# zhengfei0908/SBA-GAN

Measured on AMD Instinct MI355X. Metric: images/sec (G+D step) at 256px, higher is better.
Workload: dtype bf16; 1 GPU; bird_style.yml 3-stage G+D step (64..256px), B=20 per GPU, G_NET variant=model, image_encoder=inception, text_encoder=RNN_ENCODER in the step; global_batch=20, parallelism=dp1, launch=replayer, losses_finite=True

## Files before the change

### sba-gan_amd/csrc/norm_act.hip

```cpp
#include "common.h"

namespace {

constexpr float LRELU_SLOPE = 0.2f;


template <int ACT>
__device__ __forceinline__ float bn_act_elem(float ya, float sca, float sha, float yg, float scg, float shg) {
    const float n = ya * sca + sha;
    if (ACT == SBA_ACT_GLU) return n * sigmoidf_(yg * scg + shg);
    if (ACT == SBA_ACT_LRELU) return n > 0.f ? n : LRELU_SLOPE * n;
    if (ACT == SBA_ACT_RELU) return fmaxf(n, 0.f);
    return n;
}

struct ChCoef { float scale, shift, mean, rstd; };
__device__ __forceinline__ void ch_coef_pair(const float* __restrict__ scale, const float* __restrict__ shift,
                                             const float* __restrict__ mean, const float* __restrict__ rstd, int ca, int cg,
                                             ChCoef& ka, ChCoef& kg) {
    ka.scale = scale[ca]; ka.shift = shift[ca]; kg.scale = scale[cg]; kg.shift = shift[cg];
    ka.mean = mean[ca]; ka.rstd = rstd[ca]; kg.mean = mean[cg]; kg.rstd = rstd[cg];
}
template <int ACT>
__device__ __forceinline__ void bn_bwd_elem(float ya, float yg, float dd, const ChCoef& ka, const ChCoef& kg,
                                            float (&dz)[2], float (&xh)[2]) {
    if (ACT == SBA_ACT_GLU) {
        const float n = ya * ka.scale + ka.shift;
        const float gp = yg * kg.scale + kg.shift;
        const float s = sigmoid_bwd_(gp);
        dz[0] = dd * s;
        dz[1] = dd * n * s * (1.f - s);
    } else {
        dz[0] = dd;
        if (ACT == SBA_ACT_LRELU) {
            const float n = ya * ka.scale + ka.shift;
            dz[0] = n > 0.f ? dd : LRELU_SLOPE * dd;
        }
    }
    xh[0] = (ya - ka.mean) * ka.rstd;
    if (ACT == SBA_ACT_GLU) xh[1] = (yg - kg.mean) * kg.rstd;
}

struct Moments { float mean, var, rstd; };
__device__ __forceinline__ Moments moments_of(float sum, float sumsq, float count, float eps) {
    Moments m;
    m.mean = sum / count;
    m.var = fmaxf(sumsq / count - m.mean * m.mean, 0.f);
    m.rstd = rsqrtf(m.var + eps);
    return m;
}
struct BnCoef { float scale, shift, mean, rstd, var; };
__device__ __forceinline__ BnCoef bn_affine(float mean, float var, float rstd, float gamma, float beta) {
    BnCoef k;
    k.mean = mean; k.var = var; k.rstd = rstd;
    k.scale = gamma * rstd;
    k.shift = beta - mean * k.scale;
    return k;
}
__device__ __forceinline__ void store_aux(float* __restrict__ aux, int C, int c, const BnCoef& k) {
    aux[c] = k.scale; aux[C + c] = k.shift; aux[2 * C + c] = k.mean; aux[3 * C + c] = k.rstd;
}
__device__ __forceinline__ void running_update(float& rm, float& rv, float mean, float var, float count, float momentum) {
    const float unb = count > 1.f ? var * count / (count - 1.f) : var;
    rm = (1.f - momentum) * rm + momentum * mean;
    rv = (1.f - momentum) * rv + momentum * unb;
}
__device__ __forceinline__ BnCoef bn_coef(const float* __restrict__ stats, const float* __restrict__ gamma,
                                          const float* __restrict__ beta, int C, int c, float count, float eps) {
    float s0 = 0.f, s1 = 0.f;
#pragma unroll
    for (int sl = 0; sl < SBA_BN_STAT_SLOTS; ++sl) {
        s0 += stats[sl * 2 * C + c];
        s1 += stats[sl * 2 * C + C + c];
    }
    const Moments m = moments_of(s0, s1, count, eps);
    return bn_affine(m.mean, m.var, m.rstd, gamma[c], beta[c]);
}

struct ChannelSum {
    float* acc;
    int C;
    bool det;
    __device__ __forceinline__ void clear() const {
        if (det) return;
        for (int i = threadIdx.x; i < 2 * C; i += blockDim.x) acc[i] = 0.f;
        __syncthreads();
    }
    template <int V>
    __device__ __forceinline__ void add(int tr, int c, const float (&s0)[V], const float (&s1)[V]) const {
        float* row = acc + (det ? tr * 2 * C : 0);
#pragma unroll
        for (int k = 0; k < V; ++k) {
            if (det) {
                row[c + k] = s0[k];
                row[C + c + k] = s1[k];
            } else {
                atomicAdd(&row[c + k], s0[k]);
                atomicAdd(&row[C + c + k], s1[k]);
            }
        }
    }
    template <typename Dst>
    __device__ __forceinline__ void finish(int rpi, Dst dst) const {
        __syncthreads();
        for (int i = threadIdx.x; i < 2 * C; i += blockDim.x) {
            float v = det ? 0.f : acc[i];
            if (det)
                for (int r = 0; r < rpi; ++r) v += acc[r * 2 * C + i];
            dst(i, v);
        }
    }
};

template <int NV, int V>
__device__ __forceinline__ void wave_sums_to_lds(const float (&s0)[NV][V], const float (&s1)[NV][V],
                                                 float (&s_red)[4][2 * NV * V]) {
    const int lane = threadIdx.x & 63, wid = threadIdx.x >> 6;
#pragma unroll
    for (int h = 0; h < NV; ++h)
#pragma unroll
        for (int k = 0; k < V; ++k) {
            const float a0 = wave_sum(s0[h][k]), a1 = wave_sum(s1[h][k]);
            if (lane == 0) { s_red[wid][(h * V + k) * 2] = a0; s_red[wid][(h * V + k) * 2 + 1] = a1; }
        }
    __syncthreads();
}
template <int W>
__device__ __forceinline__ float four_wave_sum(const float (&s_red)[4][W], int i) {
    return s_red[0][i] + s_red[1][i] + s_red[2][i] + s_red[3][i];
}

template <typename T>
__global__ __launch_bounds__(256) void bn_stats_kernel(const T* __restrict__ y_all, float* __restrict__ stats_all, int64_t rows, int C,
                                                       float* __restrict__ det_part) {
    constexpr int V = Vec16<T>::N;
    const T* y = y_all + (int64_t)blockIdx.y * rows * C;
    float* stats = stats_all + ((int64_t)blockIdx.y * SBA_BN_STAT_SLOTS + (blockIdx.x & (SBA_BN_STAT_SLOTS - 1))) * 2 * C;
    const int cv = C / V;
    extern __shared__ float s_acc[];
    const ChannelSum cs{s_acc, C, det_part != nullptr};
    cs.clear();
    const int tpr = cv < (int)blockDim.x ? cv : (int)blockDim.x;
    const int rpi = blockDim.x / tpr;
    const int tc = threadIdx.x % tpr, tr = threadIdx.x / tpr;
    for (int cvi = tc; cvi < cv && tr < rpi; cvi += tpr) {
        const int c = cvi * V;
        float s0[V], s1[V];
#pragma unroll
        for (int k = 0; k < V; ++k) s0[k] = s1[k] = 0.f;
        for (int64_t row = (int64_t)blockIdx.x * rpi + tr; row < rows; row += (int64_t)gridDim.x * rpi) {
            Vec16<T> a = ld16(y + row * C + c);
#pragma unroll
            for (int k = 0; k < V; ++k) { const float v = a.get(k); s0[k] += v; s1[k] += v * v; }
        }
        cs.add(tr, c, s0, s1);
    }
    float* part = det_part ? det_part + ((int64_t)blockIdx.y * gridDim.x + blockIdx.x) * 2 * C : nullptr;
    cs.finish(rpi, [&](int i, float v) {
        if (det_part) part[i] = v;
        else atomicAdd(&stats[i], v);
    });
}

template <typename T, typename YT, int ACT>
__global__ __launch_bounds__(256) void bn_act_fwd_kernel(const YT* __restrict__ y_all, const float* __restrict__ stats_all,
                                  const float* __restrict__ gamma, const float* __restrict__ beta,
                                  float* __restrict__ rmean, float* __restrict__ rvar, int64_t* __restrict__ nbt,
                                  float* __restrict__ aux_all, const T* __restrict__ residual_all,
                                  T* __restrict__ out_all, int64_t rows, int C, int out_cstride, int out_coff,
                                  float eps, float momentum, int training) {
    constexpr int V = Vec16<T>::N;
    extern __shared__ float s_co[];
    const int g = blockIdx.y;
    const int Co = ACT == SBA_ACT_GLU ? C / 2 : C;
    const float count = (float)rows;
    float* aux = aux_all + (int64_t)g * 4 * C;
    for (int c = threadIdx.x; c < C; c += blockDim.x) {
        BnCoef k;
        if (training) {
            k = bn_coef(stats_all + (int64_t)g * SBA_BN_STAT_SLOTS * 2 * C, gamma, beta, C, c, count, eps);
        } else {
            k = bn_affine(rmean[c], rvar[c], rsqrtf(rvar[c] + eps), gamma[c], beta[c]);
        }
        s_co[c] = k.scale;
        s_co[C + c] = k.shift;
        if (blockIdx.x == 0) store_aux(aux, C, c, k);
        if (blockIdx.x == 0 && g == 0 && training && rmean) {
            float rm = rmean[c], rv = rvar[c];
            for (int gg = 0; gg < (int)gridDim.y; ++gg) {
                const BnCoef q = bn_coef(stats_all + (int64_t)gg * SBA_BN_STAT_SLOTS * 2 * C, gamma, beta, C, c, count, eps);
                running_update(rm, rv, q.mean, q.var, count, momentum);
            }
            rmean[c] = rm;
            rvar[c] = rv;
        }
    }
    if (blockIdx.x == 0 && g == 0 && threadIdx.x == 0 && training && nbt) *nbt += gridDim.y;
    __syncthreads();
    const float* scale = s_co;
    const float* shift = s_co + C;
    const YT* y = y_all + (int64_t)g * rows * C;
    const T* residual = ACT != SBA_ACT_GLU && residual_all ? residual_all + (int64_t)g * rows * Co : nullptr;
    T* out = out_all + (int64_t)g * rows * out_cstride;
    const int cv = Co / V;
    const int64_t total = rows * cv;
    for (int64_t i = blockIdx.x * (int64_t)blockDim.x + threadIdx.x; i < total;
         i += (int64_t)gridDim.x * blockDim.x) {
        const int64_t row = i / cv;
        const int c = (int)(i - row * cv) * V;
        Vec16<YT> a = ld16(y + row * C + c);
        Vec16<YT> gt = ACT == SBA_ACT_GLU ? ld16(y + row * C + Co + c) : a;
        Vec16<T> r, o;
        if (residual) r = ld16(residual + row * Co + c);
// ... 107 lines not shown
        }
        return;
    }
    for (int i = threadIdx.x; i < 2 * C; i += blockDim.x) atomicAdd(&red[i], s_acc[i]);
}

template <typename T, typename YT, int ACT>
__global__ __launch_bounds__(256) void bn_bwd_apply_kernel(const YT* __restrict__ y_all, const T* __restrict__ dout_all,
                                    const float* __restrict__ aux_all, const float* __restrict__ red_all,
                                    T* __restrict__ dy_all, float* __restrict__ dgamma, float* __restrict__ dbeta,
                                    int64_t rows, int C, int dcs, int dco) {
    constexpr int V = Vec16<T>::N;
    extern __shared__ float s_k[];
    const int g = blockIdx.y;
    const float* aux = aux_all + (int64_t)g * 4 * C;
    const float* red = red_all + (int64_t)g * SBA_BN_STAT_SLOTS * 2 * C;
    const float inv = 1.f / (float)rows;
    for (int c = threadIdx.x; c < C; c += blockDim.x) {
        s_k[c] = aux[c]; s_k[C + c] = aux[C + c]; s_k[2 * C + c] = aux[2 * C + c]; s_k[3 * C + c] = aux[3 * C + c];
        float r0 = 0.f, r1 = 0.f;
#pragma unroll
        for (int sl = 0; sl < SBA_BN_STAT_SLOTS; ++sl) {
            r0 += red[(int64_t)sl * 2 * C + c];
            r1 += red[(int64_t)sl * 2 * C + C + c];
        }
        s_k[4 * C + c] = r0 * inv;
        s_k[5 * C + c] = r1 * inv;
        if (blockIdx.x == 0 && dgamma) {
            atomicAdd(&dgamma[c], r1);
            atomicAdd(&dbeta[c], r0);
        }
    }
    __syncthreads();
    const float* scale = s_k;
    const float* shift = s_k + C;
    const float* mean = s_k + 2 * C;
    const float* rstd = s_k + 3 * C;
    const float* P = s_k + 4 * C;
    const float* Q = s_k + 5 * C;
    const YT* y = y_all + (int64_t)g * rows * C;
    const T* dout = dout_all + (int64_t)g * rows * dcs;
    T* dy = dy_all + (int64_t)g * rows * C;
    const int Co = ACT == SBA_ACT_GLU ? C / 2 : C;
    const int cv = Co / V;
    const int64_t total = rows * cv;
    for (int64_t i = blockIdx.x * (int64_t)blockDim.x + threadIdx.x; i < total;
         i += (int64_t)gridDim.x * blockDim.x) {
        const int64_t row = i / cv;
        const int c = (int)(i - row * cv) * V;
        Vec16<YT> a = ld16(y + row * C + c);
        Vec16<T> d = ld16(dout + row * dcs + dco + c);
        Vec16<T> o;
        if (ACT == SBA_ACT_GLU) {
            Vec16<YT> gt = ld16(y + row * C + Co + c);
            Vec16<T> og;
#pragma unroll
            for (int k = 0; k < V; ++k) {
                const int ca = c + k, cg = Co + c + k;
                float dz[2], xh[2];
                ChCoef ka, kg;
                ch_coef_pair(scale, shift, mean, rstd, ca, cg, ka, kg);
                bn_bwd_elem<ACT>(a.get(k), gt.get(k), d.get(k), ka, kg, dz, xh);
                o.set(k, scale[ca] * (dz[0] - P[ca] - xh[0] * Q[ca]));
                og.set(k, scale[cg] * (dz[1] - P[cg] - xh[1] * Q[cg]));
            }
            st16(dy + row * C + Co + c, og);
        } else {
#pragma unroll
            for (int k = 0; k < V; ++k) {
                const int ca = c + k;
                float dz = d.get(k);
                if (ACT == SBA_ACT_LRELU) {
                    const float n = a.get(k) * scale[ca] + shift[ca];
                    dz = n > 0.f ? dz : LRELU_SLOPE * dz;
                }
                const float xa = (a.get(k) - mean[ca]) * rstd[ca];
                o.set(k, scale[ca] * (dz - P[ca] - xa * Q[ca]));
            }
        }
        st16(dy + row * C + c, o);
    }
}

template <typename T, typename YT, int ACT>
__global__ __launch_bounds__(256) void bn_fwd_fused_kernel(const YT* __restrict__ y_all, const float* __restrict__ gamma,
                                                           const float* __restrict__ beta, float* __restrict__ rmean,
                                                           float* __restrict__ rvar, int64_t* __restrict__ nbt,
                                                           float* __restrict__ aux_all, T* __restrict__ out_all,
                                                           int64_t rows, int groups, int C, int out_cstride,
                                                           int out_coff, float eps, float momentum) {
    constexpr int V = Vec16<T>::N;
    constexpr int NV = ACT == SBA_ACT_GLU ? 2 : 1;
    __shared__ float s_red[4][2 * NV * V];
    __shared__ float s_co[2 * NV * V];
    const int tid = threadIdx.x;
    const int Co = ACT == SBA_ACT_GLU ? C / 2 : C;
    const int c = blockIdx.x * V;
    const float count = (float)rows;
    if (blockIdx.x == 0 && tid == 0 && nbt) *nbt += groups;
    for (int g = 0; g < groups; ++g) {
        const YT* y = y_all + (int64_t)g * rows * C;
        T* out = out_all + (int64_t)g * rows * out_cstride;
        float* aux = aux_all + (int64_t)g * 4 * C;
        float s0[NV][V], s1[NV][V];
#pragma unroll
        for (int h = 0; h < NV; ++h)
#pragma unroll
            for (int k = 0; k < V; ++k) { s0[h][k] = 0.f; s1[h][k] = 0.f; }
        for (int64_t row = tid; row < rows; row += 256) {
#pragma unroll
            for (int h = 0; h < NV; ++h) {
                Vec16<YT> a = ld16(y + row * C + c + h * Co);
#pragma unroll
                for (int k = 0; k < V; ++k) { const float v = a.get(k); s0[h][k] += v; s1[h][k] += v * v; }
            }
        }
        wave_sums_to_lds(s0, s1, s_red);
        if (tid < NV * V) {
            const int h = tid / V, k = tid - h * V, ch = c + h * Co + k;
            const Moments m = moments_of(four_wave_sum(s_red, tid * 2), four_wave_sum(s_red, tid * 2 + 1), count, eps);
            const BnCoef q = bn_affine(m.mean, m.var, m.rstd, gamma[ch], beta[ch]);
            s_co[tid * 2] = q.scale;
            s_co[tid * 2 + 1] = q.shift;
            store_aux(aux, C, ch, q);
            if (rmean) running_update(rmean[ch], rvar[ch], q.mean, q.var, count, momentum);
        }
        __syncthreads();
        for (int64_t row = tid; row < rows; row += 256) {
            Vec16<YT> a = ld16(y + row * C + c);
            Vec16<YT> gt = ACT == SBA_ACT_GLU ? ld16(y + row * C + Co + c) : a;
            Vec16<T> o;
#pragma unroll
            for (int k = 0; k < V; ++k) {
                const int kg = (NV - 1) * V + k;
                o.set(k, bn_act_elem<ACT>(a.get(k), s_co[k * 2], s_co[k * 2 + 1], gt.get(k), s_co[kg * 2], s_co[kg * 2 + 1]));
            }
            st16(out + row * out_cstride + out_coff + c, o);
        }
        __syncthreads();
    }
}

template <typename T, typename YT, int ACT>
__global__ __launch_bounds__(256) void bn_bwd_fused_kernel(const YT* __restrict__ y_all, const T* __restrict__ dout_all,
                                                           const float* __restrict__ aux_all, T* __restrict__ dy_all,
                                                           float* __restrict__ dgamma, float* __restrict__ dbeta,
                                                           int64_t rows, int C, int dcs, int dco) {
    constexpr int V = Vec16<T>::N;
    constexpr int NV = ACT == SBA_ACT_GLU ? 2 : 1;
    __shared__ float s_red[4][2 * NV * V];
    __shared__ float s_tot[2 * NV * V];
    const int g = blockIdx.y, tid = threadIdx.x;
    const int Co = ACT == SBA_ACT_GLU ? C / 2 : C;
    const int c = blockIdx.x * V;
    const YT* y = y_all + (int64_t)g * rows * C;
    const T* dout = dout_all + (int64_t)g * rows * dcs;
    T* dy = dy_all + (int64_t)g * rows * C;
    const float* aux = aux_all + (int64_t)g * 4 * C;
    ChCoef kc[NV][V];
#pragma unroll
    for (int k = 0; k < V; ++k)
        ch_coef_pair(aux, aux + C, aux + 2 * C, aux + 3 * C, c + k, c + (NV - 1) * Co + k, kc[0][k], kc[NV - 1][k]);
    float s0[NV][V], s1[NV][V];
#pragma unroll
    for (int h = 0; h < NV; ++h)
#pragma unroll
        for (int k = 0; k < V; ++k) { s0[h][k] = 0.f; s1[h][k] = 0.f; }
    auto dz_row = [&](int64_t row, float (&dz)[NV][V], float (&xh)[NV][V]) {
        Vec16<YT> a = ld16(y + row * C + c);
        Vec16<T> d = ld16(dout + row * dcs + dco + c);
        Vec16<YT> gt = ACT == SBA_ACT_GLU ? ld16(y + row * C + Co + c) : a;
#pragma unroll
        for (int k = 0; k < V; ++k) {
            float z[2], x[2];
            bn_bwd_elem<ACT>(a.get(k), gt.get(k), d.get(k), kc[0][k], kc[NV - 1][k], z, x);
#pragma unroll
            for (int h = 0; h < NV; ++h) { dz[h][k] = z[h]; xh[h][k] = x[h]; }
        }
    };
    for (int64_t row = tid; row < rows; row += 256) {
        float dz[NV][V], xh[NV][V];
        dz_row(row, dz, xh);
#pragma unroll
        for (int h = 0; h < NV; ++h)
#pragma unroll
            for (int k = 0; k < V; ++k) { s0[h][k] += dz[h][k]; s1[h][k] += dz[h][k] * xh[h][k]; }
    }
    wave_sums_to_lds(s0, s1, s_red);
    if (tid < 2 * NV * V) s_tot[tid] = four_wave_sum(s_red, tid);
    __syncthreads();
    if (tid < NV * V && dgamma) {
        const int h = tid / V, k = tid - h * V;
        atomicAdd(&dgamma[c + h * Co + k], s_tot[tid * 2 + 1]);
        atomicAdd(&dbeta[c + h * Co + k], s_tot[tid * 2]);
    }
    const float inv = 1.f / (float)rows;
    for (int64_t row = tid; row < rows; row += 256) {
        float dz[NV][V], xh[NV][V];
        dz_row(row, dz, xh);
#pragma unroll
        for (int h = 0; h < NV; ++h) {
            Vec16<T> o;
#pragma unroll
            for (int k = 0; k < V; ++k)
                o.set(k, kc[h][k].scale * (dz[h][k] - s_tot[(h * V + k) * 2] * inv - xh[h][k] * s_tot[(h * V + k) * 2 + 1] * inv));
            st16(dy + row * C + c + h * Co, o);
        }
    }
}

constexpr int BN1D_BM = 32;
template <bool CACHED, typename T, int N>
__device__ __forceinline__ float sample_at(const float (&cache)[N], const T* __restrict__ p, int stride, int col, int b) {
    if constexpr (CACHED) return cache[b];
    else return to_f<T>(p[(int64_t)b * stride + col]);
}
#define BN1D_EACH_SAMPLE(b, B, CACHED) \
    _Pragma("unroll CACHED ? BN1D_BM : 1") for (int b = 0; b < (CACHED ? BN1D_BM : B); ++b) if (b < B)

template <typename T, bool CACHED>
__device__ __forceinline__ void bn1d_glu_fwd_body(const float* __restrict__ y, const float* __restrict__ gamma,
                                                  const float* __restrict__ beta, float* __restrict__ rmean,
                                                  float* __restrict__ rvar, float* __restrict__ mean_o,
                                                  float* __restrict__ rstd_o, T* __restrict__ out, int B, int F, int f,
                                                  float eps, float momentum) {
    const int fh = F / 2, Cg = fh / 16;
    float yv[2][CACHED ? BN1D_BM : 1];
    if constexpr (CACHED) {
#pragma unroll
        for (int b = 0; b < BN1D_BM; ++b) {
            yv[0][b] = b < B ? y[(int64_t)b * F + f] : 0.f;
            yv[1][b] = b < B ? y[(int64_t)b * F + f + fh] : 0.f;
        }
    }
    float sc[2], sh[2];
#pragma unroll
    for (int h = 0; h < 2; ++h) {
        const int ff = f + h * fh;
        float s = 0.f, q = 0.f;
        BN1D_EACH_SAMPLE(b, B, CACHED) s += sample_at<CACHED>(yv[h], y, F, ff, b);
        const float mean = s / B;
        BN1D_EACH_SAMPLE(b, B, CACHED) { const float v = sample_at<CACHED>(yv[h], y, F, ff, b) - mean; q += v * v; }
        const float var = q / B, r = rsqrtf(var + eps);
        sc[h] = gamma[ff] * r; sh[h] = beta[ff] - mean * sc[h];
        mean_o[ff] = mean; rstd_o[ff] = r;
        if (rmean) running_update(rmean[ff], rvar[ff], mean, var, (float)B, momentum);
    }
    const int c = f / 16, s16 = f % 16;
    BN1D_EACH_SAMPLE(b, B, CACHED) {
        const float ya = sample_at<CACHED>(yv[0], y, F, f, b), yg = sample_at<CACHED>(yv[1], y, F, f + fh, b);
        const float n = fmaf(ya, sc[0], sh[0]), gp = fmaf(yg, sc[1], sh[1]);
        out[((int64_t)b * 16 + s16) * Cg + c] = from_f<T>(n * sigmoidf_(gp));
    }
}

template <typename T>
__global__ __launch_bounds__(256) void bn1d_glu_fwd_kernel(const float* __restrict__ y, const float* __restrict__ gamma,
                                    const float* __restrict__ beta, float* __restrict__ rmean,
                                    float* __restrict__ rvar, int64_t* __restrict__ nbt,
                                    float* __restrict__ mean_o, float* __restrict__ rstd_o,
                                    T* __restrict__ out, int B, int F, float eps, float momentum) {
    const int f = blockIdx.x * blockDim.x + threadIdx.x;
    if (f == 0 && nbt) *nbt += 1;
    if (f >= F / 2) return;
    if (B <= BN1D_BM) bn1d_glu_fwd_body<T, true>(y, gamma, beta, rmean, rvar, mean_o, rstd_o, out, B, F, f, eps, momentum);
    else bn1d_glu_fwd_body<T, false>(y, gamma, beta, rmean, rvar, mean_o, rstd_o, out, B, F, f, eps, momentum);
}

struct Bn1dCoef { float scale, beta, mean, rstd; };
__device__ __forceinline__ void bn1d_glu_dz(float ya, float yg, float dd, const Bn1dCoef& ka, const Bn1dCoef& kg,
                                            float& dza, float& dzg) {
    const float n = (ya - ka.mean) * ka.scale + ka.beta, gp = (yg - kg.mean) * kg.scale + kg.beta, s = sigmoidf_(gp);
    dza = dd * s;
    dzg = dd * n * s * (1.f - s);
}

template <typename T, bool CACHED>
__device__ __forceinline__ void bn1d_glu_bwd_body(const float* __restrict__ y, const T* __restrict__ dout,
                                                  const float* __restrict__ gamma, const float* __restrict__ beta,
                                                  const float* __restrict__ mean, const float* __restrict__ rstd,
                                                  float* __restrict__ dy, float* __restrict__ dgamma,
                                                  float* __restrict__ dbeta, int B, int F, int f) {
    const int fh = F / 2, Cg = fh / 16;
    const int fa = f, fg = f + fh, dcol = (f % 16) * Cg + f / 16;
    const Bn1dCoef ka{gamma[fa] * rstd[fa], beta[fa], mean[fa], rstd[fa]}, kg{gamma[fg] * rstd[fg], beta[fg], mean[fg], rstd[fg]};
    constexpr int NB = CACHED ? BN1D_BM : 1;
    float ya_[NB], yg_[NB], dd_[NB];
    if constexpr (CACHED) {
// ... 71 lines not shown
    const int n = blockIdx.x, tc = blockIdx.y, tid = threadIdx.x;
    const T* base = h + (int64_t)n * HW * C + tc * V;
    float s0[V], s1[V];
#pragma unroll
    for (int k = 0; k < V; ++k) s0[k] = s1[k] = 0.f;
    int p = tid;
    for (; p + 3 * 256 < HW; p += 4 * 256) {
        Vec16<T> a0 = ld16(base + (int64_t)p * C), a1 = ld16(base + (int64_t)(p + 256) * C);
        Vec16<T> a2 = ld16(base + (int64_t)(p + 512) * C), a3 = ld16(base + (int64_t)(p + 768) * C);
#pragma unroll
        for (int k = 0; k < V; ++k) {
            const float v0 = a0.get(k), v1 = a1.get(k), v2 = a2.get(k), v3 = a3.get(k);
            s0[k] += (v0 + v1) + (v2 + v3);
            s1[k] += (v0 * v0 + v1 * v1) + (v2 * v2 + v3 * v3);
        }
    }
    for (; p < HW; p += 256) {
        Vec16<T> a = ld16(base + (int64_t)p * C);
#pragma unroll
        for (int k = 0; k < V; ++k) { const float v = a.get(k); s0[k] += v; s1[k] += v * v; }
    }
    __shared__ float s_part[4][2 * V];
#pragma unroll
    for (int k = 0; k < V; ++k) {
        const float a = wave_sum(s0[k]), b = wave_sum(s1[k]);
        if ((tid & 63) == 0) { s_part[tid >> 6][k] = a; s_part[tid >> 6][V + k] = b; }
    }
    __syncthreads();
    if (tid < V) {
        const float sm = (s_part[0][tid] + s_part[1][tid]) + (s_part[2][tid] + s_part[3][tid]);
        const float sq = (s_part[0][V + tid] + s_part[1][V + tid]) + (s_part[2][V + tid] + s_part[3][V + tid]);
        const Moments m = moments_of(sm, sq, (float)HW, eps);
        mean[n * C + tc * V + tid] = m.mean;
        rstd[n * C + tc * V + tid] = m.rstd;
    }
}

__global__ __launch_bounds__(256) void instnorm_finalize_kernel(float* __restrict__ mean, float* __restrict__ rstd, int NC,
                                         float HW, float eps) {
    const int i = blockIdx.x * blockDim.x + threadIdx.x;
    if (i >= NC) return;
    const Moments m = moments_of(mean[i], rstd[i], HW, eps);
    mean[i] = m.mean;
    rstd[i] = m.rstd;
}

template <typename T>
__global__ __launch_bounds__(256) void adain_fwd_kernel(const T* __restrict__ h, const float* __restrict__ mean,
                                 const float* __restrict__ rstd, const float* __restrict__ style,
                                 T* __restrict__ out, int N, int HW, int C, int ocs, int oco) {
    constexpr int V = Vec16<T>::N;
    const int cv = C / V;
    const int64_t total = (int64_t)N * HW * cv;
    for (int64_t i = blockIdx.x * (int64_t)blockDim.x + threadIdx.x; i < total;
         i += (int64_t)gridDim.x * blockDim.x) {
        const int64_t row = i / cv;
        const int c = (int)(i - row * cv) * V;
        const int n = (int)(row / HW);
        Vec16<T> a = ld16(h + row * C + c), o;
#pragma unroll
        for (int k = 0; k < V; ++k) {
            const float xh = (a.get(k) - mean[n * C + c + k]) * rstd[n * C + c + k];
            o.set(k, (style[n * 2 * C + c + k] + 1.f) * xh + style[n * 2 * C + C + c + k]);
        }
        st16(out + row * ocs + oco + c, o);
    }
}

template <typename T>
__global__ __launch_bounds__(256) void adain_bwd_reduce_kernel(const T* __restrict__ h, const T* __restrict__ dout,
                                        const float* __restrict__ mean, const float* __restrict__ rstd,
                                        float* __restrict__ red, int HW, int C, int dcs, int dco, int det) {
    constexpr int V = Vec16<T>::N;
    const int cv = C / V, n = blockIdx.x;
    const int rpi = blockDim.x / cv;
    const int tc = threadIdx.x % cv, tr = threadIdx.x / cv;
    extern __shared__ float s_acc[];
    const ChannelSum cs{s_acc, C, det != 0};
    cs.clear();
    float s0[V], s1[V];
#pragma unroll
    for (int k = 0; k < V; ++k) s0[k] = s1[k] = 0.f;
    if (tr < rpi) {
        for (int p = blockIdx.y * rpi + tr; p < HW; p += gridDim.y * rpi) {
            const int64_t row = (int64_t)n * HW + p;
            Vec16<T> a = ld16(h + row * C + tc * V);
            Vec16<T> d = ld16(dout + row * dcs + dco + tc * V);
#pragma unroll
            for (int k = 0; k < V; ++k) {
                const int c = tc * V + k;
                const float xh = (a.get(k) - mean[n * C + c]) * rstd[n * C + c];
                s0[k] += d.get(k) * xh;
                s1[k] += d.get(k);
            }
        }
        cs.add(tr, tc * V, s0, s1);
    }
    cs.finish(rpi, [&](int i, float v) {
        float* dst = i < C ? &red[(n * C + i) * 2 + 0] : &red[(n * C + i - C) * 2 + 1];
        if (det) *dst += v;
        else atomicAdd(dst, v);
    });
}

template <typename T>
__global__ __launch_bounds__(256) void adain_bwd_apply_kernel(const T* __restrict__ h, const T* __restrict__ dout,
                                       const float* __restrict__ mean, const float* __restrict__ rstd,
                                       const float* __restrict__ style, const float* __restrict__ red,
                                       T* __restrict__ dh, float* __restrict__ dstyle, int N, int HW,
                                       int C, int dcs, int dco, int accumulate) {
    constexpr int V = Vec16<T>::N;
    const int cv = C / V;
    const float inv = 1.f / HW;
    if (blockIdx.x == 0 && dstyle) {
        for (int i = threadIdx.x; i < N * C; i += blockDim.x) {
            const int n = i / C, c = i - n * C;
            dstyle[n * 2 * C + c] = red[i * 2 + 0];
            dstyle[n * 2 * C + C + c] = red[i * 2 + 1];
        }
    }
    const int64_t total = (int64_t)N * HW * cv;
    for (int64_t i = blockIdx.x * (int64_t)blockDim.x + threadIdx.x; i < total;
         i += (int64_t)gridDim.x * blockDim.x) {
        const int64_t row = i / cv;
        const int c = (int)(i - row * cv) * V;
        const int n = (int)(row / HW);
        Vec16<T> a = ld16(h + row * C + c);
        Vec16<T> d = ld16(dout + row * dcs + dco + c);
        Vec16<T> o;
        if (accumulate) o = ld16(dh + row * C + c);
#pragma unroll
        for (int k = 0; k < V; ++k) {
            const int nc = n * C + c + k;
            const float xh = (a.get(k) - mean[nc]) * rstd[nc];
            const float g = (style[n * 2 * C + c + k] + 1.f) * rstd[nc];
            float v = g * (d.get(k) - red[nc * 2 + 1] * inv - xh * red[nc * 2 + 0] * inv);
            if (accumulate) v += o.get(k);
            o.set(k, v);
        }
        st16(dh + row * C + c, o);
    }
}

inline int grid_for(int64_t items, int cap = 4096) {
    int64_t b = (items + 255) / 256;
    if (b < 1) b = 1;
    return (int)(b > cap ? cap : b);
}
inline bool pow2(int v) { return v > 0 && (v & (v - 1)) == 0; }

inline int vec_width(int dtype) { return dtype != SBA_F32 ? 8 : 4; }
inline int64_t elem_size(int dtype) { return dtype != SBA_F32 ? 2 : 4; }
inline bool slice_ok(int stride, int offset, int width, int V) {
    return stride >= width + offset && stride % V == 0 && offset % V == 0;
}
inline int act_width(int C, int act) { return act == SBA_ACT_GLU ? C / 2 : C; }

constexpr int BN_RED_WORKGROUPS = 512;
constexpr int BN_RED_WORKGROUPS_PER_GROUP = 64;
struct ReduceGrid { int rpi, blocks; };
inline ReduceGrid reduce_grid(int64_t rows, int cv, int groups) {
    ReduceGrid r;
    r.rpi = cv < 256 ? 256 / cv : 1;
    r.blocks = cdiv(rows, (int64_t)r.rpi * 8);
    const int cap = BN_RED_WORKGROUPS / groups > BN_RED_WORKGROUPS_PER_GROUP ? BN_RED_WORKGROUPS / groups
                                                                              : BN_RED_WORKGROUPS_PER_GROUP;
    if (r.blocks > cap) r.blocks = cap;
    if (r.blocks < 1) r.blocks = 1;
    return r;
}
template <typename Launch>
int reduce_pass(int groups, ReduceGrid rg, int C, float* dst, hipStream_t st, Launch launch) {
    float* part = nullptr;
    size_t sh = 2 * (size_t)C * sizeof(float);
    if (sba_det_on()) {
        part = sba_det_alloc((int64_t)groups * rg.blocks * 2 * C);
        if (!part) return SBA_E_ARG;
        sh *= rg.rpi;
    }
    const int rc = launch(sh, part);
    if (rc != SBA_OK) return rc;
    if (part) sba_det_fold(part, groups, rg.blocks, 2 * C, dst, (int64_t)SBA_BN_STAT_SLOTS * 2 * C, 0, st);
    return SBA_CHECK_LAUNCH();
}
template <typename Launch>
int param_grad_pass(int groups, bool param_grads, Launch launch) {
    const int step = sba_det_on() && groups > 1 && param_grads ? 1 : groups;
    for (int g = 0; g < groups; g += step) {
        const int rc = launch(g, step);
        if (rc != SBA_OK) return rc;
    }
    return SBA_CHECK_LAUNCH();
}
inline int instnorm_splits(int HW, int rpi, bool det) {
    const int splits = cdiv(HW, rpi * 16);
    return det ? 1 : splits > 256 ? 256 : splits;
}

}

extern "C" int sba_bn_stats(int dtype, const void* y, float* stats, int64_t rows, int groups, int C,
                            void* stream) {
    const int V = vec_width(dtype);
    if (!y || !stats || rows <= 0 || groups <= 0 || groups > 65535 || C <= 0 || C % V || C > 4096)
        return SBA_E_ARG;
    const ReduceGrid rg = reduce_grid(rows, C / V, groups);
    return reduce_pass(groups, rg, C, stats, (hipStream_t)stream, [&](size_t sh, float* part) -> int {
        SBA_DISPATCH_Y(dtype, SBA_LAUNCH((bn_stats_kernel<YT>), dim3(rg.blocks, groups), dim3(256), sh, (hipStream_t)stream,
                                         (const YT*)y, stats, rows, C, part));
        return SBA_OK;
    });
}

#define ACT_CASE(A, ...) case A: { constexpr int ACT = A; __VA_ARGS__; } break;
#define ACT_SWITCH_(act, EXTRA_CASE, ...)                                                                       \
    switch (act) {                                                                                               \
        ACT_CASE(SBA_ACT_NONE, __VA_ARGS__) ACT_CASE(SBA_ACT_GLU, __VA_ARGS__) ACT_CASE(SBA_ACT_LRELU, __VA_ARGS__) \
        EXTRA_CASE                                                                                               \
        default: return SBA_E_ARG;                                                                               \
    }
#define ACT_SWITCH(act, ...) ACT_SWITCH_(act, , __VA_ARGS__)
#define ACT_SWITCH_FWD(act, ...) ACT_SWITCH_(act, ACT_CASE(SBA_ACT_RELU, __VA_ARGS__), __VA_ARGS__)

static bool bn_shape_ok(int dtype, int64_t rows, int groups, int C, int act) {
    return rows > 0 && groups > 0 && groups <= 65535 && C > 0 && pow2(C) && act_width(C, act) % vec_width(dtype) == 0 &&
           C <= 4096;
}

extern "C" int sba_bn_act_fwd(int dtype, const void* y, const float* stats, const float* gamma,
                              const float* beta, float* running_mean, float* running_var,
                              int64_t* num_batches_tracked, float* aux, const void* residual, void* out,
                              int64_t rows, int groups, int C, int act, int out_cstride, int out_coff, float eps,
                              float momentum, int training, void* stream) {
    const int V = vec_width(dtype), Co = act_width(C, act);
    const bool shape_ok = rows > 0 && groups > 0 && groups <= 65535 && C > 0 && C <= 4096 &&
                          (act == SBA_ACT_GLU ? Co % V == 0 && C % 2 == 0 : C % V == 0);
    if (!y || !gamma || !beta || !aux || !out || !shape_ok) return SBA_E_ARG;
    if (training ? !stats : (!running_mean || !running_var)) return SBA_E_ARG;
    if ((running_mean == nullptr) != (running_var == nullptr)) return SBA_E_ARG;
    if (act == SBA_ACT_GLU && residual) return SBA_E_ARG;
    if (!slice_ok(out_cstride, out_coff, Co, V)) return SBA_E_ARG;
    const int blocks = grid_for(rows * (Co / V));
    const size_t sh = 2 * (size_t)C * sizeof(float);
    SBA_DISPATCH_Y(dtype, ACT_SWITCH_FWD(act, SBA_LAUNCH((bn_act_fwd_kernel<T, YT, ACT>), dim3(blocks, groups),
                                                               dim3(256), sh, (hipStream_t)stream, (const YT*)y, stats,
                                                               gamma, beta, running_mean, running_var,
                                                               num_batches_tracked, aux, (const T*)residual, (T*)out,
                                                               rows, C, out_cstride, out_coff, eps, momentum,
                                                               training)));
    return SBA_CHECK_LAUNCH();
}

extern "C" int sba_bn_act_bwd_reduce(int dtype, const void* y, const void* dout, const float* aux, float* red,
                                     int64_t rows, int groups, int C, int act, int dcs, int dco, void* stream) {
    if (!y || !dout || !aux || !red || !bn_shape_ok(dtype, rows, groups, C, act)) return SBA_E_ARG;
    const int V = vec_width(dtype), Co = act_width(C, act);
    if (!slice_ok(dcs, dco, Co, V)) return SBA_E_ARG;
    const ReduceGrid rg = reduce_grid(rows, Co / V, groups);
    return reduce_pass(groups, rg, C, red, (hipStream_t)stream, [&](size_t sh, float* part) -> int {
        SBA_DISPATCH_Y(dtype, ACT_SWITCH(act, SBA_LAUNCH((bn_bwd_reduce_kernel<T, YT, ACT>), dim3(rg.blocks, groups),
                                                               dim3(256), sh, (hipStream_t)stream, (const YT*)y,
                                                               (const T*)dout, aux, red, rows, C, dcs, dco, part)));
        return SBA_OK;
    });
}

extern "C" int sba_bn_act_bwd_apply(int dtype, const void* y, const void* dout, const float* aux,
                                    const float* red, void* dy, float* dgamma, float* dbeta, int64_t rows,
                                    int groups, int C, int act, int dcs, int dco, void* stream) {
    if (!y || !dout || !aux || !red || !dy || !bn_shape_ok(dtype, rows, groups, C, act)) return SBA_E_ARG;
    if ((dgamma == nullptr) != (dbeta == nullptr)) return SBA_E_ARG;
    const int V = vec_width(dtype), Co = act_width(C, act);
    if (!slice_ok(dcs, dco, Co, V)) return SBA_E_ARG;
    const int blocks = grid_for(rows * (Co / V));
    const size_t sh = 6 * (size_t)C * sizeof(float);
    const int64_t esz = elem_size(dtype);
    return param_grad_pass(groups, dgamma != nullptr, [&](int g, int ng) -> int {
        const char* yg = (const char*)y + (int64_t)g * rows * C * esz;
        const char* dg = (const char*)dout + (int64_t)g * rows * dcs * esz;
        char* dyg = (char*)dy + (int64_t)g * rows * C * esz;
        const float* auxg = aux + (int64_t)g * 4 * C;
        const float* redg = red + (int64_t)g * SBA_BN_STAT_SLOTS * 2 * C;
        SBA_DISPATCH_Y(dtype, ACT_SWITCH(act, SBA_LAUNCH((bn_bwd_apply_kernel<T, YT, ACT>), dim3(blocks, ng), dim3(256), sh,
                                                               (hipStream_t)stream, (const YT*)yg, (const T*)dg, auxg, redg,
                                                               (T*)dyg, dgamma, dbeta, rows, C, dcs, dco)));
        return SBA_OK;
    });
}

extern "C" int sba_bn_act_fwd_fused(int dtype, const void* y, const float* gamma, const float* beta,
                                    float* running_mean, float* running_var, int64_t* num_batches_tracked,
                                    float* aux, void* out, int64_t rows, int groups, int C, int act,
                                    int out_cstride, int out_coff, float eps, float momentum, void* stream) {
    if (!y || !gamma || !beta || !aux || !out || !bn_shape_ok(dtype, rows, groups, C, act)) return SBA_E_ARG;
    if ((running_mean == nullptr) != (running_var == nullptr)) return SBA_E_ARG;
    const int V = vec_width(dtype), Co = act_width(C, act);
    if (!slice_ok(out_cstride, out_coff, Co, V)) return SBA_E_ARG;
    SBA_DISPATCH_Y(dtype, ACT_SWITCH(act, SBA_LAUNCH((bn_fwd_fused_kernel<T, YT, ACT>), dim3(Co / V), dim3(256), 0,
                                                           (hipStream_t)stream, (const YT*)y, gamma, beta,
                                                           running_mean, running_var, num_batches_tracked, aux,
                                                           (T*)out, rows, groups, C, out_cstride, out_coff, eps,
                                                           momentum)));
    return SBA_CHECK_LAUNCH();
}

extern "C" int sba_bn_act_bwd_fused(int dtype, const void* y, const void* dout, const float* aux, void* dy,
                                    float* dgamma, float* dbeta, int64_t rows, int groups, int C, int act, int dcs,
                                    int dco, void* stream) {
    if (!y || !dout || !aux || !dy || !bn_shape_ok(dtype, rows, groups, C, act)) return SBA_E_ARG;
    if ((dgamma == nullptr) != (dbeta == nullptr)) return SBA_E_ARG;
    const int V = vec_width(dtype), Co = act_width(C, act);
    if (!slice_ok(dcs, dco, Co, V)) return SBA_E_ARG;
    const int64_t esz = elem_size(dtype);
    return param_grad_pass(groups, dgamma != nullptr, [&](int g, int ng) -> int {
        const char* yg = (const char*)y + (int64_t)g * rows * C * esz;
        const char* dg = (const char*)dout + (int64_t)g * rows * dcs * esz;
        char* dyg = (char*)dy + (int64_t)g * rows * C * esz;
        const float* auxg = aux + (int64_t)g * 4 * C;
        SBA_DISPATCH_Y(dtype, ACT_SWITCH(act, SBA_LAUNCH((bn_bwd_fused_kernel<T, YT, ACT>), dim3(Co / V, ng), dim3(256), 0,
                                                               (hipStream_t)stream, (const YT*)yg, (const T*)dg, auxg,
                                                               (T*)dyg, dgamma, dbeta, rows, C, dcs, dco)));
        return SBA_OK;
    });
}

extern "C" int sba_bn1d_glu_fwd(int dtype, const float* y, const float* gamma, const float* beta,
                                float* running_mean, float* running_var, int64_t* nbt, float* mean, float* rstd,
                                void* out, int B, int F, float eps, float momentum, void* stream) {
    if (!y || !gamma || !beta || !mean || !rstd || !out || B <= 0 || F <= 0 || F % 32 != 0) return SBA_E_ARG;
    if ((running_mean == nullptr) != (running_var == nullptr)) return SBA_E_ARG;
    SBA_DISPATCH(dtype, SBA_LAUNCH((bn1d_glu_fwd_kernel<T>), dim3(cdiv(F / 2, 64)), dim3(64), 0,
                                           (hipStream_t)stream, y, gamma, beta, running_mean, running_var, nbt,
                                           mean, rstd, (T*)out, B, F, eps, momentum));
    return SBA_CHECK_LAUNCH();
}

extern "C" int sba_bn1d_glu_bwd(int dtype, const float* y, const void* dout, const float* gamma, const float* beta,
                                const float* mean, const float* rstd, float* dy, float* dgamma, float* dbeta,
                                int B, int F, void* stream) {
    if (!y || !dout || !gamma || !beta || !mean || !rstd || !dy || !dgamma || !dbeta || B <= 0 || F <= 0 ||
        F % 32 != 0)
        return SBA_E_ARG;
    SBA_DISPATCH(dtype, SBA_LAUNCH((bn1d_glu_bwd_kernel<T>), dim3(cdiv(F / 2, 64)), dim3(64), 0,
                                           (hipStream_t)stream, y, (const T*)dout, gamma, beta, mean, rstd, dy,
                                           dgamma, dbeta, B, F));
    return SBA_CHECK_LAUNCH();
}

static bool in_shape_ok(int dtype, int N, int HW, int C) {
    if (dtype != SBA_F32 && dtype != SBA_BF16) return false;
    const int V = vec_width(dtype);
    return N > 0 && HW > 0 && C > 0 && C % V == 0 && C / V <= 256 && pow2(C / V);
}

extern "C" int sba_instnorm_stats(int dtype, const void* h, float* mean, float* rstd, int N, int HW, int C,
                                  float eps, void* stream) {
    if (!h || !mean || !rstd || !in_shape_ok(dtype, N, HW, C)) return SBA_E_ARG;
    hipStream_t st = (hipStream_t)stream;
    const int V = vec_width(dtype);
    if (N * (C / V) >= 64 && HW >= 1024) {
        SBA_DISPATCH(dtype, SBA_LAUNCH((instnorm_stats_fused_kernel<T>), dim3(N, C / V), dim3(256), 0, st, (const T*)h, mean,
                                               rstd, HW, C, eps));
        return SBA_CHECK_LAUNCH();
    }
    sba_zero_f32(mean, rstd, (int64_t)N * C, st);
    const int rpi = 256 / (C / V);
    const bool det = sba_det_on();
    SBA_DISPATCH(dtype, SBA_LAUNCH((instnorm_accum_kernel<T>), dim3(N, instnorm_splits(HW, rpi, det)), dim3(256),
                                           (det ? rpi : 1) * 2 * C * sizeof(float), st, (const T*)h, mean, rstd, HW, C,
                                           (int)det));
    SBA_LAUNCH(instnorm_finalize_kernel, dim3(cdiv(N * C, 256)), dim3(256), 0, st, mean, rstd, N * C,
                       (float)HW, eps);
    return SBA_CHECK_LAUNCH();
}


extern "C" int sba_adain_fwd(int dtype, const void* h, const float* mean, const float* rstd, const float* style,
                             void* out, int N, int HW, int C, int ocs, int oco, void* stream) {
    if (!h || !mean || !rstd || !style || !out || !in_shape_ok(dtype, N, HW, C)) return SBA_E_ARG;
    const int V = vec_width(dtype);
    if (!slice_ok(ocs, oco, C, V)) return SBA_E_ARG;
    const int blocks = grid_for((int64_t)N * HW * (C / V));
    SBA_DISPATCH(dtype, SBA_LAUNCH((adain_fwd_kernel<T>), dim3(blocks), dim3(256), 0, (hipStream_t)stream,
                                           (const T*)h, mean, rstd, style, (T*)out, N, HW, C, ocs, oco));
    return SBA_CHECK_LAUNCH();
}

extern "C" int sba_adain_bwd_reduce(int dtype, const void* h, const void* dout, const float* mean,
                                    const float* rstd, float* red, int N, int HW, int C, int dcs, int dco,
                                    void* stream) {
    if (!h || !dout || !mean || !rstd || !red || !in_shape_ok(dtype, N, HW, C)) return SBA_E_ARG;
    const int V = vec_width(dtype);
    if (!slice_ok(dcs, dco, C, V)) return SBA_E_ARG;
    const int rpi = 256 / (C / V);
    const bool det = sba_det_on();
    SBA_DISPATCH(dtype, SBA_LAUNCH((adain_bwd_reduce_kernel<T>), dim3(N, instnorm_splits(HW, rpi, det)), dim3(256),
                                           (det ? rpi : 1) * 2 * C * sizeof(float), (hipStream_t)stream, (const T*)h,
                                           (const T*)dout, mean, rstd, red, HW, C, dcs, dco, (int)det));
    return SBA_CHECK_LAUNCH();
}

extern "C" int sba_adain_bwd_apply(int dtype, const void* h, const void* dout, const float* mean,
                                   const float* rstd, const float* style, const float* red, void* dh,
                                   float* dstyle, int N, int HW, int C, int dcs, int dco, int accumulate,
// ... 11 lines not shown
```

Measured before the change: 2114 images/sec.

## Cache BN rows in registers across fused passes and prefetch AdaIN reduce rows

The fused batchnorm+activation forward and backward kernels now load each thread's rows once into a register array (up to 10 rows, chosen by a row-count switch), then reuse them for both the statistics pass and the normalize/gradient pass. Global memory is read once instead of twice when the row count is small. The AdaIN backward reduction now issues four row loads before consuming them, keeping more memory requests in flight. In exchange, register pressure and template instantiations grow, which may lower occupancy. The backward output formula is also rewritten with explicit rounding control to keep numerics stable.

```diff
diff --git a/sba-gan_amd/csrc/norm_act.hip b/sba-gan_amd/csrc/norm_act.hip
--- a/sba-gan_amd/csrc/norm_act.hip
+++ b/sba-gan_amd/csrc/norm_act.hip
@@ -41,6 +41,11 @@
     if (ACT == SBA_ACT_GLU) xh[1] = (yg - kg.mean) * kg.rstd;
 }
 
+__device__ __forceinline__ float mul_rn(float a, float b) {
+#pragma clang fp contract(off)
+    return a * b;
+}
+
 struct Moments { float mean, var, rstd; };
 __device__ __forceinline__ Moments moments_of(float sum, float sumsq, float count, float eps) {
     Moments m;
@@ -129,6 +134,26 @@
 __device__ __forceinline__ float four_wave_sum(const float (&s_red)[4][W], int i) {
     return s_red[0][i] + s_red[1][i] + s_red[2][i] + s_red[3][i];
 }
+
+template <int D, typename Load, typename Use>
+__device__ __forceinline__ void rows_in_flight(int64_t row0, int64_t stride, int64_t rows, Load load, Use use) {
+    decltype(load(row0)) v[D];
+    int64_t row = row0;
+    for (; row + (D - 1) * stride < rows; row += D * stride) {
+#pragma unroll
+        for (int s = 0; s < D; ++s) v[s] = load(row + s * stride);
+#pragma unroll
+        for (int s = 0; s < D; ++s) use(v[s]);
+    }
+    if (row < rows) {
+#pragma unroll
+        for (int s = 0; s < D; ++s) { const int64_t r = row + s * stride; v[s] = load(r < rows ? r : rows - 1); }
+#pragma unroll
+        for (int s = 0; s < D; ++s)
+            if (row + s * stride < rows) use(v[s]);
+    }
+}
+constexpr int ADAIN_REDUCE_DEPTH = 4;
 
 template <typename T>
 __global__ __launch_bounds__(256) void bn_stats_kernel(const T* __restrict__ y_all, float* __restrict__ stats_all, int64_t rows, int C,
@@ -402,7 +427,23 @@
     }
 }
 
-template <typename T, typename YT, int ACT>
+constexpr int BN_FUSED_CACHE_ROWS = 10;
+constexpr int BN_FUSED_CACHE_ROWS_MID = 5;
+constexpr int BN_FUSED_CACHE_ROWS_SMALL = 2;
+#define BN_EACH_OWN_ROW(i, row, rows, R)                                                                              \
+    _Pragma("unroll R ? R : 1") for (int i = 0; i < (R ? R : (int)(((rows) - threadIdx.x + 255) / 256)); ++i)             \
+        if (const int64_t row = threadIdx.x + (int64_t)i * 256; row < (rows))
+__device__ __forceinline__ int64_t own_row_clamped(int tid, int i, int64_t rows) {
+    const int64_t row = tid + (int64_t)i * 256;
+    return row < rows ? row : rows - 1;
+}
+template <int R, typename U, int N>
+__device__ __forceinline__ Vec16<U> own_row(const Vec16<U> (&cache)[N], const U* __restrict__ p, int i) {
+    if constexpr (R > 0) return cache[i];
+    else return ld16(p);
+}
+
+template <typename T, typename YT, int ACT, int R>
 __global__ __launch_bounds__(256) void bn_fwd_fused_kernel(const YT* __restrict__ y_all, const float* __restrict__ gamma,
                                                            const float* __restrict__ beta, float* __restrict__ rmean,
                                                            float* __restrict__ rvar, int64_t* __restrict__ nbt,
@@ -427,10 +468,20 @@
         for (int h = 0; h < NV; ++h)
 #pragma unroll
             for (int k = 0; k < V; ++k) { s0[h][k] = 0.f; s1[h][k] = 0.f; }
-        for (int64_t row = tid; row < rows; row += 256) {
+        Vec16<YT> yc[NV][R ? R : 1];
+        if constexpr (R > 0) {
+#pragma unroll
+            for (int i = 0; i < R; ++i)
+#pragma unroll
+                for (int h = 0; h < NV; ++h) {
+                    const int64_t row = own_row_clamped(tid, i, rows);
+                    yc[h][i] = ld16(y + row * C + c + h * Co);
+                }
+        }
+        BN_EACH_OWN_ROW(i, row, rows, R) {
 #pragma unroll
             for (int h = 0; h < NV; ++h) {
-                Vec16<YT> a = ld16(y + row * C + c + h * Co);
+                Vec16<YT> a = own_row<R>(yc[h], y + row * C + c + h * Co, i);
 #pragma unroll
                 for (int k = 0; k < V; ++k) { const float v = a.get(k); s0[h][k] += v; s1[h][k] += v * v; }
             }
@@ -446,9 +497,9 @@
             if (rmean) running_update(rmean[ch], rvar[ch], q.mean, q.var, count, momentum);
         }
         __syncthreads();
-        for (int64_t row = tid; row < rows; row += 256) {
-            Vec16<YT> a = ld16(y + row * C + c);
-            Vec16<YT> gt = ACT == SBA_ACT_GLU ? ld16(y + row * C + Co + c) : a;
+        BN_EACH_OWN_ROW(i, row, rows, R) {
+            Vec16<YT> a = own_row<R>(yc[0], y + row * C + c, i);
+            Vec16<YT> gt = ACT == SBA_ACT_GLU ? own_row<R>(yc[NV - 1], y + row * C + Co + c, i) : a;
             Vec16<T> o;
 #pragma unroll
             for (int k = 0; k < V; ++k) {
@@ -461,7 +512,7 @@
     }
 }
 
-template <typename T, typename YT, int ACT>
+template <typename T, typename YT, int ACT, int R>
 __global__ __launch_bounds__(256) void bn_bwd_fused_kernel(const YT* __restrict__ y_all, const T* __restrict__ dout_all,
                                                            const float* __restrict__ aux_all, T* __restrict__ dy_all,
                                                            float* __restrict__ dgamma, float* __restrict__ dbeta,
@@ -486,10 +537,18 @@
     for (int h = 0; h < NV; ++h)
 #pragma unroll
         for (int k = 0; k < V; ++k) { s0[h][k] = 0.f; s1[h][k] = 0.f; }
-    auto dz_row = [&](int64_t row, float (&dz)[NV][V], float (&xh)[NV][V]) {
-        Vec16<YT> a = ld16(y + row * C + c);
-        Vec16<T> d = ld16(dout + row * dcs + dco + c);
-        Vec16<YT> gt = ACT == SBA_ACT_GLU ? ld16(y + row * C + Co + c) : a;
+    Vec16<YT> yc[NV][R ? R : 1];
+    Vec16<T> dc[R ? R : 1];
+    if constexpr (R > 0) {
+#pragma unroll
+        for (int i = 0; i < R; ++i) {
+            const int64_t row = own_row_clamped(tid, i, rows);
+            yc[0][i] = ld16(y + row * C + c);
+            dc[i] = ld16(dout + row * dcs + dco + c);
+            if (ACT == SBA_ACT_GLU) yc[NV - 1][i] = ld16(y + row * C + Co + c);
+        }
+    }
+    auto dz_row = [&](const Vec16<YT>& a, const Vec16<T>& d, const Vec16<YT>& gt, float (&dz)[NV][V], float (&xh)[NV][V]) {
 #pragma unroll
         for (int k = 0; k < V; ++k) {
             float z[2], x[2];
@@ -498,9 +557,12 @@
             for (int h = 0; h < NV; ++h) { dz[h][k] = z[h]; xh[h][k] = x[h]; }
         }
     };
-    for (int64_t row = tid; row < rows; row += 256) {
+    BN_EACH_OWN_ROW(i, row, rows, R) {
+        Vec16<YT> a = own_row<R>(yc[0], y + row * C + c, i);
+        Vec16<T> d = own_row<R>(dc, dout + row * dcs + dco + c, i);
+        Vec16<YT> gt = ACT == SBA_ACT_GLU ? own_row<R>(yc[NV - 1], y + row * C + Co + c, i) : a;
         float dz[NV][V], xh[NV][V];
-        dz_row(row, dz, xh);
+        dz_row(a, d, gt, dz, xh);
 #pragma unroll
         for (int h = 0; h < NV; ++h)
 #pragma unroll
@@ -515,15 +577,19 @@
         atomicAdd(&dbeta[c + h * Co + k], s_tot[tid * 2]);
     }
     const float inv = 1.f / (float)rows;
-    for (int64_t row = tid; row < rows; row += 256) {
+    BN_EACH_OWN_ROW(i, row, rows, R) {
+        Vec16<YT> a = own_row<R>(yc[0], y + row * C + c, i);
+        Vec16<T> d = own_row<R>(dc, dout + row * dcs + dco + c, i);
+        Vec16<YT> gt = ACT == SBA_ACT_GLU ? own_row<R>(yc[NV - 1], y + row * C + Co + c, i) : a;
         float dz[NV][V], xh[NV][V];
-        dz_row(row, dz, xh);
+        dz_row(a, d, gt, dz, xh);
 #pragma unroll
         for (int h = 0; h < NV; ++h) {
             Vec16<T> o;
 #pragma unroll
             for (int k = 0; k < V; ++k)
-                o.set(k, kc[h][k].scale * (dz[h][k] - s_tot[(h * V + k) * 2] * inv - xh[h][k] * s_tot[(h * V + k) * 2 + 1] * inv));
+                o.set(k, kc[h][k].scale * fmaf(-mul_rn(xh[h][k], s_tot[(h * V + k) * 2 + 1]), inv,
+                                               dz[h][k] - mul_rn(s_tot[(h * V + k) * 2], inv)));
             st16(dy + row * C + c + h * Co, o);
         }
     }
@@ -761,18 +827,20 @@
 #pragma unroll
     for (int k = 0; k < V; ++k) s0[k] = s1[k] = 0.f;
     if (tr < rpi) {
-        for (int p = blockIdx.y * rpi + tr; p < HW; p += gridDim.y * rpi) {
+        struct Row { Vec16<T> a, d; };
+        const auto load = [&](int64_t p) {
             const int64_t row = (int64_t)n * HW + p;
-            Vec16<T> a = ld16(h + row * C + tc * V);
-            Vec16<T> d = ld16(dout + row * dcs + dco + tc * V);
+            return Row{ld16(h + row * C + tc * V), ld16(dout + row * dcs + dco + tc * V)};
+        };
+        rows_in_flight<ADAIN_REDUCE_DEPTH>(blockIdx.y * rpi + tr, gridDim.y * rpi, HW, load, [&](const Row& r) {
 #pragma unroll
             for (int k = 0; k < V; ++k) {
                 const int c = tc * V + k;
-                const float xh = (a.get(k) - mean[n * C + c]) * rstd[n * C + c];
-                s0[k] += d.get(k) * xh;
-                s1[k] += d.get(k);
+                const float xh = (r.a.get(k) - mean[n * C + c]) * rstd[n * C + c];
+                s0[k] += r.d.get(k) * xh;
+                s1[k] += r.d.get(k);
             }
-        }
+        });
         cs.add(tr, tc * V, s0, s1);
     }
     cs.finish(rpi, [&](int i, float v) {
@@ -900,6 +968,14 @@
     }
 #define ACT_SWITCH(act, ...) ACT_SWITCH_(act, , __VA_ARGS__)
 #define ACT_SWITCH_FWD(act, ...) ACT_SWITCH_(act, ACT_CASE(SBA_ACT_RELU, __VA_ARGS__), __VA_ARGS__)
+
+#define FUSED_ROWS_SWITCH(rows, ...)                                                  \
+    do {                                                                              \
+        if ((rows) <= 256 * BN_FUSED_CACHE_ROWS_SMALL) { constexpr int R = BN_FUSED_CACHE_ROWS_SMALL; __VA_ARGS__; } \
+        else if ((rows) <= 256 * BN_FUSED_CACHE_ROWS_MID) { constexpr int R = BN_FUSED_CACHE_ROWS_MID; __VA_ARGS__; } \
+        else if ((rows) <= 256 * BN_FUSED_CACHE_ROWS) { constexpr int R = BN_FUSED_CACHE_ROWS; __VA_ARGS__; } \
+        else { constexpr int R = 0; __VA_ARGS__; }                                    \
+    } while (0)
 
 static bool bn_shape_ok(int dtype, int64_t rows, int groups, int C, int act) {
     return rows > 0 && groups > 0 && groups <= 65535 && C > 0 && pow2(C) && act_width(C, act) % vec_width(dtype) == 0 &&
@@ -975,11 +1051,11 @@
     if ((running_mean == nullptr) != (running_var == nullptr)) return SBA_E_ARG;
     const int V = vec_width(dtype), Co = act_width(C, act);
     if (!slice_ok(out_cstride, out_coff, Co, V)) return SBA_E_ARG;
-    SBA_DISPATCH_Y(dtype, ACT_SWITCH(act, SBA_LAUNCH((bn_fwd_fused_kernel<T, YT, ACT>), dim3(Co / V), dim3(256), 0,
-                                                           (hipStream_t)stream, (const YT*)y, gamma, beta,
-                                                           running_mean, running_var, num_batches_tracked, aux,
-                                                           (T*)out, rows, groups, C, out_cstride, out_coff, eps,
-                                                           momentum)));
+    SBA_DISPATCH_Y(dtype, ACT_SWITCH(act, FUSED_ROWS_SWITCH(rows, SBA_LAUNCH((bn_fwd_fused_kernel<T, YT, ACT, R>), dim3(Co / V),
+                                                                             dim3(256), 0, (hipStream_t)stream, (const YT*)y,
+                                                                             gamma, beta, running_mean, running_var,
+                                                                             num_batches_tracked, aux, (T*)out, rows, groups,
+                                                                             C, out_cstride, out_coff, eps, momentum))));
     return SBA_CHECK_LAUNCH();
 }
 
@@ -996,9 +1072,11 @@
         const char* dg = (const char*)dout + (int64_t)g * rows * dcs * esz;
         char* dyg = (char*)dy + (int64_t)g * rows * C * esz;
         const float* auxg = aux + (int64_t)g * 4 * C;
-        SBA_DISPATCH_Y(dtype, ACT_SWITCH(act, SBA_LAUNCH((bn_bwd_fused_kernel<T, YT, ACT>), dim3(Co / V, ng), dim3(256), 0,
-                                                               (hipStream_t)stream, (const YT*)yg, (const T*)dg, auxg,
-                                                               (T*)dyg, dgamma, dbeta, rows, C, dcs, dco)));
+        SBA_DISPATCH_Y(dtype, ACT_SWITCH(act, FUSED_ROWS_SWITCH(rows, SBA_LAUNCH((bn_bwd_fused_kernel<T, YT, ACT, R>),
+                                                                                 dim3(Co / V, ng), dim3(256), 0,
+                                                                                 (hipStream_t)stream, (const YT*)yg,
+                                                                                 (const T*)dg, auxg, (T*)dyg, dgamma, dbeta,
+                                                                                 rows, C, dcs, dco))));
         return SBA_OK;
     });
 }
```

Result: no change. 2124 images/sec (median of 3 runs) (+0.4%).
